# Intsights/PySubstringSearch

Hardware: AMD Instinct MI355X
Metric: queries/sec (batched) + index-build GB/s on 512MB chunk, 1/2/4/8 GPU (higher is better)
Workload: dtype u64

## Files before the change

include/pss.h:

```cpp
#ifndef PSS_H
#define PSS_H

#include <stddef.h>
#include <stdint.h>

#ifdef __cplusplus
extern "C" {
#endif

#define PSS_OK 0
#define PSS_EINVAL (-1)
#define PSS_ENOMEM (-2)
#define PSS_EIO (-3)
#define PSS_ETOOBIG (-4)
#define PSS_EDEVICE (-5)
#define PSS_EFORMAT (-6)

typedef struct pss_writer pss_writer;
typedef struct pss_reader pss_reader;
typedef struct pss_result pss_result;


int pss_device_count(void);

// ... 39 lines not shown
    uint64_t fs_launches[9];
    uint64_t fs_elems[9];
    uint64_t msd;
    uint64_t msd_buckets;
    uint64_t msd_max_bucket;
    uint64_t msd_tiles;
    double msd_ms_g1;
    double msd_ms_g2;
    double msd_ms_local;
    uint64_t msd_slow_tiles;
    uint64_t runs;
    uint64_t rle;
    uint64_t rle_id_bits;
    double rle_ms_table;
    double rle_ms_reduced;
    double rle_ms_expand;
    uint64_t ss;
    uint64_t ss_buckets;
    uint64_t ss_max_bucket;
    uint64_t ss_tiles;
    uint64_t ss_samples;
    double ss_ms_sample;
    double ss_ms_g1;
    double ss_ms_g2;
    double ss_ms_local;
    double ms_initial;
    uint64_t period;
    uint64_t period_extent;
    uint64_t period_path;
    uint64_t plan_hint;
    uint64_t anchor;
    uint64_t anchor_omega;
    uint64_t anchor_w;
    uint64_t anchor_count;
    uint64_t anchor_active;
    uint64_t anchor_depth;
    uint64_t anchor_text_rounds;
    uint64_t anchor_rounds;
    uint64_t anchor_sum_active;
    uint64_t anchor_left;
    uint64_t anchor_levels;
    uint64_t probe_pairs;
    uint64_t probe_same;
    uint64_t periodic_rounds;
    uint64_t periodic_members;
    uint64_t ss_planned;
    uint64_t dup_screen;
    uint64_t ss_plan_refused;
    uint64_t ss_declined_nomem;
    uint64_t anchor_side;
    double anchor_ms;
    double ms_restarts;
    uint64_t msd_lookback;
} pss_sa_stats;

int32_t pss_sa_build(const uint8_t *T, int32_t *SA, int32_t n, int32_t device);

int32_t pss_sa_build_device(const void *d_T, void *d_SA, int32_t n, int32_t device,
                            uint32_t flags, pss_sa_stats *stats);

int32_t pss_sort_pairs_device(void *d_keys, void *d_vals, uint32_t n, int32_t key_bits, int32_t device,
                              double *ms_scatter);


int pss_writer_open(const char *path, int64_t max_chunk_len, int32_t device, pss_writer **out);
#define PSS_FORMAT_STRIPED 0x100
int pss_writer_open_format(const char *path, int64_t max_chunk_len, int32_t device, int32_t format_version,
                           pss_writer **out);
int pss_writer_open_multi(const char *path, int64_t max_chunk_len, const int32_t *devices, int32_t n_devices,
                          int32_t format_version, pss_writer **out);
int pss_writer_add_entry(pss_writer *w, const uint8_t *text, uint64_t len);
int pss_writer_add_file_lines(pss_writer *w, const char *path);
int pss_writer_dump(pss_writer *w);
int pss_writer_finalize(pss_writer *w);
int pss_writer_close(pss_writer *w);
uint64_t pss_writer_chunk_limit(const pss_writer *w);
typedef struct pss_writer_io {
    uint64_t records_mapped;
    uint64_t records_pwritten;
    uint64_t ingest_direct_bytes;
    uint64_t ingest_copied_bytes;
} pss_writer_io;
int pss_writer_io_stats(pss_writer *w, pss_writer_io *out);


int pss_reader_open(const char *path, int32_t device, int32_t shard_index, int32_t shard_count,
                    pss_reader **out);
int pss_reader_open_multi(const char *path, const int32_t *devices, int32_t n_devices, pss_reader **out);
uint64_t pss_reader_part_chunks(const pss_reader *r, uint64_t *counts, uint64_t cap);

int pss_reader_set_auto_residency(pss_reader *r, int32_t on);
int pss_reader_chunk_tiers(const pss_reader *r, uint8_t *tiers, uint64_t cap, uint64_t *auto_moves);
int pss_reader_evict_chunk(pss_reader *r, uint64_t index);
int pss_reader_promote_chunk(pss_reader *r, uint64_t index);
int pss_reader_set_low_latency(pss_reader *r, int32_t on);
int pss_reader_low_latency_stats(const pss_reader *r, uint64_t *launches, uint64_t *served);
#define PSS_ORDER_TEXT 0
#define PSS_ORDER_SA 1
int pss_reader_set_result_order(pss_reader *r, int32_t order);
int32_t pss_reader_result_order(const pss_reader *r);
int pss_reader_create(int32_t device, pss_reader **out);
int pss_reader_add_chunk_device(pss_reader *r, const void *d_text, const void *d_sa, uint32_t n);
int pss_reader_set_chunk_device(pss_reader *r, uint64_t index, const void *d_text, const void *d_sa, uint32_t n);
uint64_t pss_reader_num_chunks(const pss_reader *r);
int pss_reader_residency(const pss_reader *r, uint64_t *hbm_bytes, uint64_t *host_bytes, uint64_t *host_chunks);

// ... 127 lines not shown
```

pysubstringsearch_amd/_ffi.py:

```python
import ctypes
import os

_HERE = os.path.dirname(os.path.abspath(__file__))
LIB_PATH = os.environ.get('PSS_LIBPSS') or os.path.join(_HERE, 'libpss.so')

PSS_OK, PSS_EINVAL, PSS_ENOMEM, PSS_EIO, PSS_ETOOBIG, PSS_EDEVICE, PSS_EFORMAT = 0, -1, -2, -3, -4, -5, -6

CORPUS_LINES, CORPUS_WORDS, CORPUS_RUNS, CORPUS_PERIODIC = 0, 1, 2, 3
CORPUS_REPEAT_LINE, CORPUS_DUP_BLOCKS, CORPUS_MIXED, CORPUS_SOURCE = 4, 5, 6, 7


class SaStats(ctypes.Structure):
    _fields_ = [
        ('sigma', ctypes.c_uint32),
        ('code_bits', ctypes.c_uint32),
        ('key_chars', ctypes.c_uint32),
        ('initial_passes', ctypes.c_uint32),
        ('rounds', ctypes.c_uint32),
        ('round_passes', ctypes.c_uint32),
        ('sum_active', ctypes.c_uint64),
        ('sort_elems', ctypes.c_uint64),
        ('ms_total', ctypes.c_double),
        ('ms_sort', ctypes.c_double),
        ('sort_launches', ctypes.c_uint64),
# ... 10 lines not shown
        ('fs_launches', ctypes.c_uint64 * 9),
        ('fs_elems', ctypes.c_uint64 * 9),
        ('msd', ctypes.c_uint64),
        ('msd_buckets', ctypes.c_uint64),
        ('msd_max_bucket', ctypes.c_uint64),
        ('msd_tiles', ctypes.c_uint64),
        ('msd_ms_g1', ctypes.c_double),
        ('msd_ms_g2', ctypes.c_double),
        ('msd_ms_local', ctypes.c_double),
        ('msd_slow_tiles', ctypes.c_uint64),
        ('runs', ctypes.c_uint64),
        ('rle', ctypes.c_uint64),
        ('rle_id_bits', ctypes.c_uint64),
        ('rle_ms_table', ctypes.c_double),
        ('rle_ms_reduced', ctypes.c_double),
        ('rle_ms_expand', ctypes.c_double),
        ('ss', ctypes.c_uint64),
        ('ss_buckets', ctypes.c_uint64),
        ('ss_max_bucket', ctypes.c_uint64),
        ('ss_tiles', ctypes.c_uint64),
        ('ss_samples', ctypes.c_uint64),
        ('ss_ms_sample', ctypes.c_double),
        ('ss_ms_g1', ctypes.c_double),
        ('ss_ms_g2', ctypes.c_double),
        ('ss_ms_local', ctypes.c_double),
        ('ms_initial', ctypes.c_double),
        ('period', ctypes.c_uint64),
        ('period_extent', ctypes.c_uint64),
        ('period_path', ctypes.c_uint64),
        ('plan_hint', ctypes.c_uint64),
        ('anchor', ctypes.c_uint64),
        ('anchor_omega', ctypes.c_uint64),
        ('anchor_w', ctypes.c_uint64),
        ('anchor_count', ctypes.c_uint64),
        ('anchor_active', ctypes.c_uint64),
        ('anchor_depth', ctypes.c_uint64),
        ('anchor_text_rounds', ctypes.c_uint64),
        ('anchor_rounds', ctypes.c_uint64),
        ('anchor_sum_active', ctypes.c_uint64),
        ('anchor_left', ctypes.c_uint64),
        ('anchor_levels', ctypes.c_uint64),
        ('probe_pairs', ctypes.c_uint64),
        ('probe_same', ctypes.c_uint64),
        ('periodic_rounds', ctypes.c_uint64),
        ('periodic_members', ctypes.c_uint64),
        ('ss_planned', ctypes.c_uint64),
        ('dup_screen', ctypes.c_uint64),
        ('ss_plan_refused', ctypes.c_uint64),
        ('ss_declined_nomem', ctypes.c_uint64),
        ('anchor_side', ctypes.c_uint64),
        ('anchor_ms', ctypes.c_double),
        ('ms_restarts', ctypes.c_double),
        ('msd_lookback', ctypes.c_uint64),
    ]

    def as_dict(self):
        d = {k: getattr(self, k) for k, _ in self._fields_}
        for k in ('fs_ms', 'fs_launches', 'fs_elems'):
            d[k] = list(d[k])
        return d


def knobs():
    out = []
    for i in range(lib.pss_knob_count()):
        f = [ctypes.c_char_p() for _ in range(4)]
        check(lib.pss_knob_info(i, *[ctypes.byref(x) for x in f]))
        name, dflt, fuzz, what = [x.value.decode() for x in f]
        out.append({'name': name, 'default': dflt, 'fuzz': [v for v in fuzz.split('|') if v], 'what': what})
    return out


class SearchStats(ctypes.Structure):
    _fields_ = [
        ('queries', ctypes.c_uint64),
        ('hits', ctypes.c_uint64),
        ('entries', ctypes.c_uint64),
        ('result_bytes', ctypes.c_uint64),
        ('ms_device', ctypes.c_double),
        ('ms_interval', ctypes.c_double),
        ('ms_host', ctypes.c_double),
        ('route', ctypes.c_uint32),
        ('route_pad', ctypes.c_uint32),
    ]

    def as_dict(self):
        return {k: getattr(self, k) for k, _ in self._fields_ if k != 'route_pad'}


ROUTES = {
    'RESIDENT': 0x0001,
    'SMALL_BLOCK': 0x0002,
    'SMALL_WAVE': 0x0004,
    'SMALL_OVERFLOW': 0x0008,
    'INTERVAL_LANE': 0x0010,
    'INTERVAL_GROUP': 0x0020,
    'INTERVAL_WAVE': 0x0040,
    'KEY_SAMPLES': 0x0080,
    'MID': 0x0100,
    'MID_OVERFLOW': 0x0200,
    'GENERAL': 0x0400,
    'SA_ORDER': 0x0800,
    'COUNTS': 0x1000,
    'ANCHORED': 0x2000,
}

# ... 198 lines not shown
```

pysubstringsearch_amd/csrc/common.cpp:

```cpp
#include "common.h"
#include "knobs.h"

#include <atomic>
#include <cstring>
#include <cstdio>
#include <cstdlib>
#include <algorithm>
#include <cerrno>
#include <unistd.h>

#include <mutex>
#include <vector>

namespace pss {

static thread_local std::string g_err;

void set_error(const char *fmt, ...)
{
    char buf[1024];
    va_list ap;
    va_start(ap, fmt);
    vsnprintf(buf, sizeof buf, fmt, ap);
    va_end(ap);
// ... 325 lines not shown
    return PSS_OK;
}

int get_ctx(int device, DeviceCtx **out) { return get_ctx_of(g_ctx, device, out); }
int get_build_ctx(int device, DeviceCtx **out) { return get_ctx_of(g_bctx, device, out); }

int DeviceCtx::ensure_resident()
{
    if (resident.arena) return PSS_OK;
    PSS_HIP(hipStreamCreateWithFlags(&resident.stream, hipStreamNonBlocking));
    PSS_HIP(hipHostMalloc(&resident.arena, kPinnedBytes, hipHostMallocCoherent | hipHostMallocMapped));
    PSS_HIP(hipHostGetDevicePointer(&resident.arena_dev, resident.arena, 0));
    memset(resident.arena, 0, kPinnedBytes);
    return PSS_OK;
}

void DeviceCtx::Resident::post(const uint8_t *q, uint32_t plen)
{
    ResidentMailbox *mb = reinterpret_cast<ResidentMailbox *>(static_cast<uint8_t *>(arena) + kResidentMailboxOff);
    if (plen != kResidentStop) {
        if (plen <= sizeof mb->post.bytes) {
            memcpy(mb->post.bytes, q, plen);
        } else {
            memcpy(mb->query, q, plen);
            memset(mb->query + plen, 0, 32);
        }
    }
    mb->post.plen = plen;
    ++seq;
    __atomic_store_n(&mb->post.seq_b, seq, __ATOMIC_RELEASE);
    __atomic_store_n(&mb->post.seq_a, seq, __ATOMIC_RELEASE);
}

void DeviceCtx::stop_resident()
{
    if (!resident.running) return;
    resident.post(nullptr, kResidentStop);
    (void)hipStreamSynchronize(resident.stream);
    resident.running = false;
}

const KnobDef kKnobs[] = {
    {"PSS_KEY_CHARS", "0 (chosen)", "1|2|3|5|8|12|16", "builder: force the symbols packed into the initial sort key"},
    {"PSS_KEY_DROP", "-1 (chosen)", "0|1|3|7", "builder: force the low bits of the last key symbol that are left out"},
    {"PSS_NO_SAMPLE", "unset", "1", "builder: size the initial key from symbol counts even for large texts (no sizing sample)"},
    {"PSS_NO_TIES_PASS", "unset", "1", "builder: plain 8-byte-key LSD passes and key comparison in the rerank (no tie flags)"},
    {"PSS_MODE", "chosen", "dense|sparse|text", "builder: how ties are resolved -- doubling over an inverse suffix array, sparse (hash), text rounds"},
    {"PSS_TEXT_ROUNDS", "5", "0|1|2|3", "builder: text rounds at most before the rank rounds"},
    {"PSS_MSD", "-1 (screened)", "0|1|1", "initial sort: never / whenever the key fits the hybrid MSD radix sort (msd_sort.hip)"},
    {"PSS_MSD_LSD", "1", "0|1", "MSD sort: 0 = digits in MSD order with a second histogram pass (rounds 2-5); else LSD order, second pass by look-back"},
    {"PSS_MSD_KEY_CAP", "48", "", "MSD sort: largest key width tried (bits; the element format bounds it further)"},
    {"PSS_MSD_PARTIAL_SYMBOL", "unset", "1", "MSD sort: fill the element with the high bits of one more symbol than fits whole (fewer ties; measured slower on lines)"},
    {"PSS_MSD_NO_FUSE", "unset", "1", "MSD sort: ties flagged in the suffix array instead of emitted from the local sort"},
    {"PSS_MSD_SLOW_LOCAL", "unset", "1", "MSD sort: the general (ballot LSD) local-sort kernel for every tile"},
    {"PSS_MSD_SCATTER", "unset", "1", "MSD sort in MSD order: the 8192-element partition kernels of round 2"},
    {"PSS_SS", "-1 (n >= 2^24, MSD declined)", "0|1", "initial sort: never / whenever the text has the size for it the sample sort over 16-byte elements"},
    {"PSS_SS_SEG", "1", "0", "sample sort: 0 = every tile merge-sorted as one array instead of bucket by bucket"},
    {"PSS_SS_WINDOW_PLAN", "unset", "1", "sample sort: tiles by the window rule of the MSD sort instead of the greedy plan"},
    {"PSS_SS_DEBUG", "unset", "", "sample sort: print where a bucket beyond a tile came from (diagnostic)"},
    {"PSS_NO_PLAN_CACHE", "unset", "1", "builder: forget between chunks which initial sort and alphabet the previous chunk took"},
    {"PSS_NO_PLAN_FRONT", "unset", "1", "builder: remember the sort but not the alphabet (separate alphabet and recode passes)"},
    {"PSS_RLE", "-1 (runs average >= 8 bytes)", "0|1|1", "builder: never / always the run-length path (rle_build.hip)"},
    {"PSS_RLE_SORT", "unset", "1", "run-length path: expansion by the stable radix sort instead of the matrix walk"},
    {"PSS_PERIOD", "-1 (when the text repeats one word)", "0", "builder: 0 = never the closed form for a text that repeats one word"},
    {"PSS_ANCHOR", "-1 (texts of >= 2^20 bytes)", "0|1|1", "builder: never / whenever ties outlive the text rounds the anchor round (anchor_impl.h)"},
    {"PSS_ANCHOR_OMEGA", "0 (as wide as the common prefix allows)", "9|12|17|33", "anchor round: force the window of the minimizers"},
    {"PSS_ANCHOR_MIN_OMEGA", "11", "3|7|9", "anchor round: narrowest window it accepts by itself"},
    {"PSS_ANCHOR_SIDE", "-1 (>= 2^24 bytes, sampled ties show copies)", "0|1", "anchor round: never / always sort the anchors beside the text round (second stream)"},
    {"PSS_ANCHOR_SIDE_PCT", "8", "", "anchor round: share of sampled tied pairs that must be copies for the side line"},
    {"PSS_ANCHOR_CAP_DIV", "5", "3|4", "anchor round: declines above n / this many anchors"},
    {"PSS_NO_PROBE", "unset", "1", "builder: always a text round before the anchor round (no sampling of the ties)"},
    {"PSS_PROBE_SKIP_PCT", "50", "0|20|90", "builder: no text rounds when more than this share of the sampled tied pairs are repeats"},
    {"PSS_NO_MID_TIER", "unset", "1", "rounds: groups above 512 members all take the chained radix sorts"},
    {"PSS_NO_MID_MERGE", "unset", "1", "rounds: groups of 513 .. 4096 members with a crowded bin take the chained sorts (no LDS merge sort)"},
    {"PSS_BIG_MERGE", "-1 (by the average size of the large groups)", "0|1|2", "rounds: groups above 4096 members through the segmented merge sort (2: in text rounds only)"},
    {"PSS_NO_BIG_MERGE", "unset", "", "rounds: overrides PSS_BIG_MERGE"},
    {"PSS_COUNT_SORT", "unset", "1", "rank rounds: groups ranked by counting instead of the merge sort"},
    {"PSS_PERIODIC", "1", "0", "rank rounds: 0 = no periodic keys for the large groups"},
    {"PSS_TIMING", "unset", "", "builder / Writer: per-round and per-stage trace on stderr"},
    {"PSS_DEVICES", "all visible", "0|0,0|0,0,0|all", "devices of Reader(path) / Writer(path) without a device argument: all | comma-separated ordinals"},
    {"PSS_DEVICE", "unset", "", "default device of a process (launchers' LOCAL_RANK etc. are honoured the same way)"},
    {"PSS_IO_THREADS", "8 .. 16 by core count", "2|5", "file path: threads of the I/O pool"},
    {"PSS_INGEST_BLOCK", "32 MiB", "16|40|300", "Writer: size of the direct reads of add_entries_from_file_lines"},
    {"PSS_INGEST_MIN_ROOM", "1 MiB", "1|20", "Writer: room a chunk must have left for one direct read"},
    {"PSS_WRITER_MMAP", "tmpfs: 1, else 0", "0|1", "Writer: records through a shared mapping (1) or pwrite (0)"},
    {"PSS_WRITER_MMAP_MIN", "1 MiB", "16", "Writer: smallest record that goes through the mapping"},
    {"PSS_WRITER_HOST_BUDGET", "8 GiB", "", "multi-device Writer: host text of the chunks in flight (one chunk always goes through)"},
    {"PSS_STRIPES", "8", "", "striped container format 2: stripe files of a Writer"},
    {"PSS_EXPERIMENT_NO_FILE", "unset", "", "measurement only: the record thread copies without writing the file"},
    {"PSS_RESULT_ORDER", "text", "sa", "Reader: 'sa' = the reference's order inside a chunk (suffix-array order of every entry's first hit)"},
    {"PSS_READER_HBM_BUDGET", "whatever hipMalloc grants minus 2 GiB", "", "Reader: suffix arrays beyond this many bytes of HBM stay in pinned host memory"},
    {"PSS_READER_AUTO_RESIDENCY", "1", "", "Reader: 0 = the residency manager never moves a suffix array by itself"},
    {"PSS_NO_KEY_SAMPLES", "unset", "", "Reader: no key-sample table"},
    {"PSS_SAMPLE_SHIFT", "11", "", "Reader: one key sample per 2^shift suffixes"},
    {"PSS_LINE_BLOCK_SHIFT", "8", "6|7|9|10", "Reader: the line index behind entry ids keeps one newline rank per 2^shift bytes of text (6 .. 10)"},
    {"PSS_NO_SMALL_PATH", "unset", "1", "search: no fused single-query kernels"},
    {"PSS_NO_BLOCK_PATH", "unset", "1", "search: small batches one wave per pair instead of one workgroup"},
    {"PSS_NO_SEARCH_STAGE", "unset", "1", "search: no pinned staging of queries and results"},
    {"PSS_WAVE_SEARCH", "unset", "1", "search: interval kernel one wave per pair at every batch size"},
    {"PSS_NO_GROUP_SEARCH", "unset", "1", "search: never 16 lanes per pair"},
    {"PSS_NO_MID_PIPELINE", "unset", "1", "search: always the general multi-kernel pipeline"},
    {"PSS_PINNED_POOL_BYTES", "40 GiB", "", "search: pinned host memory the result pool keeps between batches"},
    {"PSS_NO_PINNED_RESULTS", "unset", "1", "search: large results into pageable memory"},
    {"PSS_LANE_SEARCH_MIN", "8192", "1|100000", "search: pairs from which one lane per pair searches"},
    {"PSS_ICASE_SEED_LETTERS", "5", "1|2|3|4|5|6", "case-insensitive search: ASCII letters of a pattern's seed at most (2^letters spellings probed per pattern and chunk)"},
    {"PSS_SEARCH_EVENTS", "unset", "", "single-query path: HIP events around the fused kernel (fills ms_device; ~4 us per query)"},
// ... 58 lines not shown
```

pysubstringsearch_amd/csrc/msd_sort.h:

```cpp
#pragma once
#include "common.h"
#include "radix_sort.h"

namespace pss {

struct MsdStats {
    uint32_t buckets = 0;
    uint32_t max_bucket = 0;
    uint32_t tiles = 0;
    uint32_t slow_tiles = 0;
    uint32_t bad_symbol = 0;
    uint32_t lookback = 0;
    double ms_g1 = 0, ms_g2 = 0, ms_local = 0;
};

struct MsdActive {
    uint32_t *pos, *idx, *grp;
    uint32_t *st_pos, *st_idx;
    uint32_t count = 0;
};

size_t msd_workspace_bytes(uint32_t n);
int msd_max_key_bits(uint32_t n);

struct MsdFront {
    const uint8_t *raw;
    const uint8_t *lut;
    uint32_t *bad;
};
int msd_suffix_sort(DeviceCtx *ctx, const TextKeys *text, uint32_t n, int key_bits, uint64_t *A[2], uint32_t *sa_out,
                    void *work, uint32_t *h_small, bool profile, MsdStats *stats, bool *accepted, MsdActive *active = nullptr,
                    const MsdFront *front = nullptr);


struct SsStats {
    uint32_t buckets = 0, max_bucket = 0, tiles = 0;
    uint32_t b1 = 0, b2 = 0, samples = 0;
    int key_chars = 0;
    double ms_sample = 0, ms_g1 = 0, ms_g2 = 0, ms_local = 0;
};
struct SsBuffers {
    void *A[2];
    uint16_t *digits;
    void *E0, *E;
    uint64_t *K[2];
    uint32_t *V[2];
    void *sort_work;
    const void *sample_in = nullptr;
    void *sample_keep = nullptr;
};
uint32_t ss_sample_count(uint32_t n);
int ss_key_chars(uint32_t n, uint32_t radix);
uint64_t ss_geometry_tag(uint32_t n, uint32_t radix);
int ss_suffix_sort(DeviceCtx *ctx, const TextKeys *text, uint32_t radix, uint32_t n, const SsBuffers &buf, uint32_t *sa_out,
                   void *work, uint32_t *h_small, bool profile, SsStats *stats, bool *accepted, MsdActive *active);

}
```

pysubstringsearch_amd/csrc/msd_sort.hip:

```cpp
#include "msd_sort.h"

#include <algorithm>
#include <vector>

#include "prims.h"
#include "scan.h"
#include "text_keys.h"

namespace pss {

constexpr int MSD_D = 10;
constexpr u32 MSD_BINS = 1u << MSD_D;
constexpr int MSD_BLOCK = 512;
constexpr int MSD_WAVES = MSD_BLOCK / kWave;
constexpr int MSD_IPT = 16;
constexpr u32 MSD_TILE = MSD_BLOCK * MSD_IPT;
constexpr u32 MSD_WIN = 6144;
#ifndef PSS_LS_WINDOW
#define PSS_LS_WINDOW 8
#endif
constexpr u32 MSD_TILE_CAP = 8184 - PSS_LS_WINDOW;
constexpr u32 MSD_MAX_BUCKET = 4088;
constexpr int MSD_TAG_BITS = MSD_D + 1;
constexpr u32 MSD_TAG_SPAN = 1u << MSD_TAG_BITS;
// ... 752 lines not shown
}

__global__ __launch_bounds__(256) void msd_tiles_kernel(const u32 *cstart, u32 ne, u32 n, const u64 *rank, const u64 *total,
                                                          u32 *tile_first, TilePlan tp)
{
    if (blockIdx.x == 0 && threadIdx.x == 0) tile_first[*total] = ne;
    for (u32 k = blockIdx.x * blockDim.x + threadIdx.x; k < ne; k += gridDim.x * blockDim.x) {
        if (msd_tile_head(cstart, ne, n, k, tp)) tile_first[rank[k]] = k;
    }
}

struct MsdTile {
    u32 e0, count, tag0, nb;
};


struct MsdEmit {
    u32 *st_pos, *st_idx;
    u32 *blk_cnt;
};

__device__ __forceinline__ void msd_emit_tile(const u64 *exch, u32 count, u32 e0, int idx_bits, u32 *sa_out, const MsdEmit *em,
                                              u32 *s_count)
{
    const u32 tid = threadIdx.x, lane = tid & 63u;
    const u32 imask = (u32)((1ull << idx_bits) - 1ull);
    const u32 rows = (count + MSD_BLOCK - 1) / MSD_BLOCK;
#pragma unroll 1
    for (u32 r = 0; r < rows; ++r) {
        const u32 p = r * MSD_BLOCK + tid;
        const bool valid = p < count;
        u64 x = 0;
        bool tie = false;
        if (valid) {
            x = exch[p];
            tie = p > 0 && (exch[p - 1] >> idx_bits) == (x >> idx_bits);
            sa_out[e0 + p] = ((u32)x & imask) | ((tie && em == nullptr) ? 0x80000000u : 0u);
        }
        if (em != nullptr) {
            const u64 tm = __ballot(tie);
            const bool tie_next = lane < 63 ? ((tm >> (lane + 1)) & 1ull) != 0
                                            : (p + 1 < count && (exch[p + 1] >> idx_bits) == (x >> idx_bits));
            if (valid && (tie || tie_next)) {
                const u32 slot = e0 + atomicAdd(s_count, 1u);
                em->st_pos[slot] = e0 + p;
                em->st_idx[slot] = ((u32)x & imask) | (tie ? 0x80000000u : 0u);
            }
        }
    }
}

struct InBlkCnt {
    const u32 *c;
    __device__ u64 operator()(u64 t) const { return c[t]; }
};

constexpr u32 GA_WORDS = MSD_TILE / 32;
__global__ __launch_bounds__(256) void msd_gather_kernel(const MsdTile *tiles, const u32 *blk_cnt, const u64 *dst_off, u32 nt,
                                                           const u32 *st_pos, const u32 *st_idx, u32 *pos, u32 *idx, u32 *grp)
{
    __shared__ u32 s_occ[4][GA_WORDS], s_head[4][GA_WORDS], s_pre[4][GA_WORDS];
    const u32 w = wave_id(), lane = lane_id();
    const u32 t = blockIdx.x * 4 + w;
    if (t >= nt) return;
    const u32 c = blk_cnt[t];
    if (c == 0) return;
    const u32 e0 = tiles[t].e0;
    const u64 d = dst_off[t];
    u32 *occ = s_occ[w], *head = s_head[w], *pre = s_pre[w];
    for (u32 i = lane; i < GA_WORDS; i += kWave) occ[i] = head[i] = 0;
    __builtin_amdgcn_fence(__ATOMIC_ACQ_REL, "wavefront");
    __builtin_amdgcn_wave_barrier();
    for (u32 i = lane; i < c; i += kWave) {
        const u32 q = st_pos[e0 + i] - e0;
        atomicOr(&occ[q >> 5], 1u << (q & 31u));
        if (!(st_idx[e0 + i] >> 31)) atomicOr(&head[q >> 5], 1u << (q & 31u));
    }
    __builtin_amdgcn_fence(__ATOMIC_ACQ_REL, "wavefront");
    __builtin_amdgcn_wave_barrier();
    {
        const u32 c0 = __popc(occ[4 * lane]), c1 = __popc(occ[4 * lane + 1]), c2 = __popc(occ[4 * lane + 2]),
                  c3 = __popc(occ[4 * lane + 3]);
        const u32 ex = wave_incl_sum(c0 + c1 + c2 + c3) - (c0 + c1 + c2 + c3);
        pre[4 * lane] = ex;
        pre[4 * lane + 1] = ex + c0;
        pre[4 * lane + 2] = ex + c0 + c1;
        pre[4 * lane + 3] = ex + c0 + c1 + c2;
    }
    __builtin_amdgcn_fence(__ATOMIC_ACQ_REL, "wavefront");
    __builtin_amdgcn_wave_barrier();
    for (u32 i = lane; i < c; i += kWave) {
        const u32 ps = st_pos[e0 + i], q = ps - e0;
        const u32 below = (q & 31u) ? (occ[q >> 5] & ((1u << (q & 31u)) - 1u)) : 0u;
        const u32 rank = pre[q >> 5] + __popc(below);
        u32 wi = q >> 5;
        u32 m = head[wi] & ((q & 31u) == 31u ? ~0u : ((2u << (q & 31u)) - 1u));
        while (m == 0 && wi > 0) m = head[--wi];
        const u32 hq = wi * 32 + (31u - (u32)__builtin_clz(m | 1u));
        pos[d + rank] = ps;
        idx[d + rank] = st_idx[e0 + i] & 0x7fffffffu;
        grp[d + rank] = e0 + hq + 1;
    }
}


__global__ __launch_bounds__(MSD_BLOCK) void msd_local_sort_kernel(const u64 *in, const MsdTile *tiles, int rem_bits, int idx_bits,
                                                                     u32 *sa_out, const u32 *tile_list, int fused, MsdEmit em_val)
{
    const MsdEmit *em = fused ? &em_val : nullptr;
    __shared__ __attribute__((aligned(16))) u64 exch[MSD_TILE];
    __shared__ u32 wave_hist[MSD_WAVES][256];
    __shared__ u32 scr[MSD_WAVES + 1];
    const u32 tid = threadIdx.x, lane = tid & 63u, wave = tid >> 6;
    const u32 t = tile_list ? tile_list[blockIdx.x] : blockIdx.x;
    const MsdTile td = tiles[t];
    const u32 e0 = td.e0, count = td.count;
    for (u32 i = tid; i < MSD_WAVES * 256; i += MSD_BLOCK) (&wave_hist[0][0])[i] = 0;
    __syncthreads();
    int seg_bits = 0;
    while ((1u << seg_bits) < td.nb) ++seg_bits;
    const u64 tag_base = (u64)td.tag0 << (rem_bits + idx_bits);
    u64 key[MSD_IPT];
#pragma unroll
    for (int r = 0; r < MSD_IPT; ++r) {
        const u32 p = wave * (kWave * MSD_IPT) + r * kWave + lane;
        key[r] = p < count ? in[e0 + p] - tag_base : ~0ull;
    }
    const int sort_bits = rem_bits + seg_bits;
    for (int shift = idx_bits; shift < idx_bits + sort_bits; shift += 8) {
        const int left = idx_bits + sort_bits - shift;
        const u32 dmask = left >= 8 ? 0xffu : ((1u << left) - 1u);
        u32 rank[MSD_IPT], prev[MSD_IPT];
#pragma unroll
        for (int r = 0; r < MSD_IPT; ++r) {
            const bool pad = wave * (kWave * MSD_IPT) + r * kWave + lane >= count;
            const u32 d = pad ? dmask : ((u32)(key[r] >> shift) & dmask);
            const u64 peers = match_digit8(d, ~0ull);
            const u32 below = mbcnt(peers);
            prev[r] = 0;
            if (below == 0) prev[r] = atomicAdd(&wave_hist[wave][d], (u32)__popcll(peers));
            rank[r] = below | ((u32)__builtin_ctzll(peers) << 16);
        }
#pragma unroll
        for (int r = 0; r < MSD_IPT; ++r) rank[r] = __shfl(prev[r], (int)(rank[r] >> 16)) + (rank[r] & 0xffffu);
        __syncthreads();
        {
            u32 c[MSD_WAVES];
            u32 total = 0;
            if (tid < 256) {
#pragma unroll
                for (int w = 0; w < MSD_WAVES; ++w) {
                    c[w] = wave_hist[w][tid];
                    total += c[w];
                }
            }
// ... 514 lines not shown
        else hipLaunchKernelGGL(msd_scatter_kernel<false>, dim3((u32)max_ranges2), dim3(MSD_BLOCK), 0, s, a);
        PSS_TRY(mark());
    }
    const auto local_sort = msd_local_sort_kernel;
    const auto local_fast = msd_local_fast_kernel;
    u32 nt = 0;
    u32 *fail_list = fail_list_dev;
    if (one_trip) {
        nt = h_small[8];
        if ((size_t)nt > max_tiles) {
            set_error("msd_suffix_sort: %u tiles planned, tables hold %zu (internal error)", nt, max_tiles);
            return PSS_EDEVICE;
        }
        const u32 nfail = h_small[10];
        if (stats) stats->slow_tiles = nfail;
        if (nfail)
            hipLaunchKernelGGL(local_sort, dim3(nfail), dim3(MSD_BLOCK), 0, s, A[1], (const MsdTile *)tiles_all, rem_bits,
                               ib, sa_out, (const u32 *)fail_list, fused, em);
    } else {
    const TilePlan tp{MSD_WIN, MSD_TILE_CAP, cj};
    PSS_TRY(device_excl_scan(ctx, InTileHead{cstart, ne, n, tp}, ne, partial, d_total, ranks));
    hipLaunchKernelGGL(msd_tiles_kernel, dim3(1024), dim3(256), 0, s, cstart, ne, n, ranks, (const u64 *)d_total, tile_first, tp);
    PSS_HIP(hipMemcpyAsync(h_small, d_total, 8, hipMemcpyDeviceToHost, s));
    PSS_HIP(hipStreamSynchronize(s));
    nt = h_small[0];
    if ((size_t)nt > max_tiles) {
        set_error("msd_suffix_sort: %u tiles planned, tables hold %zu (internal error)", nt, max_tiles);
        return PSS_EDEVICE;
    }
    PSS_TRY(mark());
    fail_list = tile_first + nt + 8;
    hipLaunchKernelGGL(msd_tile_desc_kernel, dim3((nt + 255) / 256), dim3(256), 0, s, cstart, tile_first, nt, ne, n, tiles_all,
                       (const u32 *)cj, (const u64 *)nullptr, (const u64 *)nullptr);
    if (knob("PSS_MSD_SLOW_LOCAL")) {
        hipLaunchKernelGGL(local_sort, dim3(nt), dim3(MSD_BLOCK), 0, s, A[1], (const MsdTile *)tiles_all, rem_bits, ib,
                           sa_out, (const u32 *)nullptr, fused, em);
    } else {
        MsdTile *tiles = tiles_all;
        const u32 grid = std::min<u32>(nt, 2u * (u32)ctx->num_cus);
        hipLaunchKernelGGL(local_fast, dim3(grid), dim3(MSD_BLOCK), 0, s, A[1], (const MsdTile *)tiles, nt, rem_bits, ib,
                           sa_out, fail_list, counters + 4, fused, em, (const u64 *)nullptr, (const u32 *)nullptr, (const u32 *)nullptr);
        PSS_TRY(mark());
        PSS_HIP(hipMemcpyAsync(h_small, counters + 4, 4, hipMemcpyDeviceToHost, s));
        PSS_HIP(hipStreamSynchronize(s));
        const u32 nfail = h_small[0];
        if (stats) stats->slow_tiles = nfail;
        if (nfail)
            hipLaunchKernelGGL(local_sort, dim3(nfail), dim3(MSD_BLOCK), 0, s, A[1], (const MsdTile *)tiles_all, rem_bits,
                               ib, sa_out, (const u32 *)fail_list, fused, em);
    }
    if (knob("PSS_MSD_SLOW_LOCAL")) PSS_TRY(mark());
    }
    if (fused) {
        PSS_TRY(device_excl_scan(ctx, InBlkCnt{blk_cnt}, nt, partial, d_total, dst_off));
        hipLaunchKernelGGL(msd_gather_kernel, dim3((nt + 3) / 4), dim3(256), 0, s, (const MsdTile *)tiles_all, blk_cnt, dst_off, nt,
                           active->st_pos, active->st_idx, active->pos, active->idx, active->grp);
        PSS_HIP(hipMemcpyAsync(h_small, d_total, 8, hipMemcpyDeviceToHost, s));
        PSS_HIP(hipStreamSynchronize(s));
        active->count = h_small[0];
    }
    PSS_HIP(hipGetLastError());
    if (stats) {
        stats->tiles = nt;
        stats->lookback = lsd ? 1u : 0u;
    }
    if (profile && nev >= 6) {
        PSS_HIP(hipStreamSynchronize(s));
        float ms = 0.f;
        PSS_HIP(hipEventElapsedTime(&ms, ev[0], ev[1]));
        if (stats) stats->ms_g1 = ms;
        PSS_HIP(hipEventElapsedTime(&ms, ev[2], ev[3]));
        if (stats) stats->ms_g2 = ms;
        PSS_HIP(hipEventElapsedTime(&ms, ev[4], ev[5]));
        if (stats) stats->ms_local = ms;
    }
    *accepted = true;
    return PSS_OK;
}


struct SsGeometry {
    u32 B1, B2, os, S;
    int ib, kc, key_bits;
    u64 plo, phi;
};
static bool ss_geometry(uint32_t n, uint32_t radix, SsGeometry *g)
{
    if (n < (1u << 16) || n > (1u << 30) || radix < 2 || radix > 257) return false;
    int ib = 1;
    while ((1ull << ib) < (u64)n) ++ib;
    const unsigned __int128 limit = (unsigned __int128)1 << (128 - ib);
    unsigned __int128 pw = 1;
    int kc = 0;
    while (kc < SS_MAX_CHARS && pw <= limit / radix) {
        pw *= radix;
        ++kc;
    }
    if (kc < 2) return false;
    unsigned __int128 lead = 1;
    for (int i = 0; i + 1 < kc; ++i) lead *= radix;
    g->plo = (u64)lead;
    g->phi = (u64)(lead >> 64);
    int kb = 0;
    while (kb < 128 && ((pw - 1) >> kb) != 0) ++kb;
    g->key_bits = kb;
    int lb = 4;
    while (((u64)512 << lb) < (u64)n && lb < 20) ++lb;
    const u32 B1 = 1u << ((lb + 1) / 2), B2 = 1u << (lb / 2);
    const u32 os = ((u64)n > (u64)768 * B1 * B2) ? 8u : 4u;
    g->B1 = B1;
    g->B2 = B2;
    g->os = os;
// ... 245 lines not shown
```

pysubstringsearch_amd/csrc/sa_build.hip:

```cpp
#include "prims.h"
#include "msd_sort.h"
#include "rle_build.h"
#include "radix_sort.h"
#include "sa_build.h"
#include "scan.h"
#include "anchor_impl.h"

#include <algorithm>
#include <cmath>
#include <string>
#include <thread>

namespace pss {


constexpr u32 DUP_SAMPLES = 8192, DUP_SLOTS = 16384;
__global__ __launch_bounds__(1024) void dup_screen_kernel(const u8 *T, u32 n, u32 *dups)
{
    __shared__ u32 table[DUP_SLOTS];
    for (u32 i = threadIdx.x; i < DUP_SLOTS; i += 1024) table[i] = 0;
    __syncthreads();
    u32 mine = 0;
    if (n >= 64) {
        const u32 stride = (n - 32) / DUP_SAMPLES;
        for (u32 k = threadIdx.x; k < DUP_SAMPLES; k += 1024) {
            u64 x = ((u64)k + 1) * 0x9E3779B97F4A7C15ull;
            x ^= x >> 29;
            x *= 0xBF58476D1CE4E5B9ull;
            x ^= x >> 32;
            const u32 pos = stride ? k * stride + (u32)(x % stride) : k % (n - 32);
            const u64 a = load_u64_unaligned(T + pos), b = load_u64_unaligned(T + pos + 8);
            u64 hsh = (a ^ (b * 0x9E3779B97F4A7C15ull)) * 0xD6E8FEB86659FD93ull;
            hsh ^= hsh >> 32;
            u32 f = (u32)hsh;
            if (f == 0) f = 1;
            u32 slot = (f * 2654435761u) >> (32 - 14);
            static_assert(DUP_SLOTS == (1u << 14), "14-bit slot");
            for (;;) {
                const u32 old = atomicCAS(&table[slot], 0u, f);
                if (old == 0u) break;
                if (old == f) { ++mine; break; }
                slot = (slot + 1) & (DUP_SLOTS - 1);
            }
        }
    }
    const u32 tot = wave_incl_sum(mine);
    if (lane_id() == kWave - 1 && tot) atomicAdd(dups, tot);
}

__global__ __launch_bounds__(256) void sa_symbols_kernel(const u8 *T, u32 n, u32 *present, u32 *counts, u32 *runs)
{
    __shared__ u32 seen[256];
    __shared__ u32 cnt[256];
    const u32 tid = threadIdx.x;
    seen[tid] = 0;
    cnt[tid] = 0;
    u32 nruns = 0;
    __syncthreads();
// ... 368 lines not shown
    const int passes0 = (key_bits0 + 7) / 8;
    const int final_buf = (passes0 - 1) & 1;
    u32 *const v_scratch = V[final_buf];
    V[final_buf] = SA;
    int cur = 0;
    const bool ties = passes0 >= 2 && !knobs.no_flags;
    bool msd_done = false, msd_fused = false;
    u32 msd_active = 0;
    if (ties && knobs.msd != 0) {
        const char *cap_env = knob("PSS_MSD_KEY_CAP");
        const int key_cap = cap_env ? atoi(cap_env) : 48;
        const bool whole = knob("PSS_MSD_PARTIAL_SYMBOL") == nullptr;
        int kb = std::min(msd_max_key_bits(n), std::max(key_cap, 21));
        int kc = std::min(whole ? kb / b : (kb + b - 1) / b, kmax);
        int mdrop = kc * b - kb;
        if (mdrop < 0 || kc <= 1) {
            kb = kc * b;
            mdrop = 0;
        }
        const bool fits = kc >= 1 && kb >= 21 && !plus_one;
        const bool auto_ok = sampled && msd_screen_ok && (hint == 1 || (key_bits0 <= 48 && kb + 8 >= key_bits0));
        if (fits && (knobs.msd == 1 || (knobs.msd < 0 && auto_ok))) {
            TextKeys mk{codes, b, kc, plus_one, mdrop};
            MsdStats ms;
            bool accepted = false;
            PSS_TRY(ctx->slot[S_GRP2].reserve((size_t)n * 4));
            MsdActive act;
            act.pos = ctx->slot[S_P1].as<u32>();
            act.idx = (final_buf == 0) ? V[1] : V[0];
            act.grp = ctx->slot[S_GRP2].as<u32>();
            act.st_pos = reinterpret_cast<u32 *>(K[0]);
            act.st_idx = reinterpret_cast<u32 *>(K[0]) + n;
            const MsdFront front{T, d_lut, d_bad};
            PSS_TRY(msd_suffix_sort(ctx, &mk, n, kb, K, SA, ctx->slot[S_P0].p, h_small, profile, &ms, &accepted,
                                    knobs.no_msd_fuse ? nullptr : &act, front_any ? &front : nullptr));
            if (front_any && !accepted) {
                ctx->plan_path = 0;
                return start_over(fresh ? (flags | 4u) : flags);
            }
            msd_fused = accepted && !knobs.no_msd_fuse;
            msd_active = act.count;
            st.msd_buckets = ms.buckets;
            st.msd_max_bucket = ms.max_bucket;
            if (accepted) {
                msd_done = true;
                key_chars = kc;
                key_drop = mdrop;
                st.key_chars = (u32)kc;
                st.key_bits = (u64)kb;
                st.msd = 1;
                st.msd_tiles = ms.tiles;
                st.msd_slow_tiles = ms.slow_tiles;
                st.msd_lookback = ms.lookback;
                st.msd_ms_g1 = ms.ms_g1;
                st.msd_ms_g2 = ms.ms_g2;
                st.msd_ms_local = ms.ms_local;
                cur = final_buf;
                ss.launches = 3;
                ss.elems = 3ull * n;
            }
        }
    }
    if (front_any && !msd_done) {
        ctx->plan_path = 0;
        return start_over(fresh ? (flags | 4u) : flags);
    }
    if (!msd_done && ties && knobs.ss != 0 && (knobs.ss == 1 || (n >= (1u << 24) && !forced_chars && knobs.key_chars == 0)) &&
        ss_sample_count(n) != 0) {
        const u32 S = ss_sample_count(n);
        bool ss_room = ctx->slot[S_SSA].reserve((size_t)n * 16 + 256) == PSS_OK && ctx->slot[S_SSB].reserve((size_t)n * 16 + 256) == PSS_OK;
        if (!ss_room) {
            (void)hipGetLastError();
            ctx->slot[S_SSA].release();
            ctx->slot[S_SSB].release();
            set_error("%s", "");
            st.ss_declined_nomem = 1;
        }
        if (ss_room) {
        PSS_TRY(ctx->slot[S_GRP2].reserve((size_t)n * 4));
        SsBuffers sb;
        sb.A[0] = ctx->slot[S_SSA].p;
        sb.A[1] = ctx->slot[S_SSB].p;
        sb.digits = reinterpret_cast<uint16_t *>(ctx->slot[S_P1].p);
        sb.E0 = GRP;
        sb.E = ISA;
        sb.K[0] = K[0]; sb.K[1] = K[1];
        sb.V[0] = v_scratch; sb.V[1] = (final_buf == 0) ? V[1] : V[0];
        sb.sort_work = work;
        const u32 radix = plus_one ? 257u : sigma + 1u;
        const u64 tag = ss_geometry_tag(n, radix);
        const bool planned = hint == 2 && tag != 0 && ctx->ss_plan_tag == tag && ctx->ss_plan_radix == radix && ctx->slot[S_SSPLAN].p != nullptr &&
                             ctx->ss_plan_skip == 0;
        if (planned) sb.sample_in = ctx->slot[S_SSPLAN].p;
        else if (plain && ctx->slot[S_SSPLAN].reserve((size_t)S * 16) == PSS_OK) sb.sample_keep = ctx->slot[S_SSPLAN].p;
        ctx->ss_plan_tag = 0;
        MsdActive act;
        act.pos = ctx->slot[S_P1].as<u32>();
        act.idx = (final_buf == 0) ? V[1] : V[0];
        act.grp = ctx->slot[S_GRP2].as<u32>();
        act.st_pos = reinterpret_cast<u32 *>(K[0]);
        act.st_idx = reinterpret_cast<u32 *>(K[0]) + n;
        TextKeys sk{codes, b, 0, plus_one, 0};
        SsStats sst;
        bool accepted = false;
        PSS_TRY(ss_suffix_sort(ctx, &sk, plus_one ? 257u : sigma + 1u, n, sb, SA, ctx->slot[S_P0].p, h_small, profile, &sst, &accepted,
                               &act));
// ... 111 lines not shown
```

pysubstringsearch_amd/csrc/sa_rerank_impl.h:

```cpp


constexpr int RR_BLOCK = 256;
constexpr int RR_WAVES = RR_BLOCK / kWave;
#ifndef PSS_RR_ROWS
#define PSS_RR_ROWS 8
#endif
constexpr int RR_ROWS = PSS_RR_ROWS;
constexpr int RR_WSEG = RR_ROWS * kWave;
constexpr int RR_TILE = RR_WSEG * RR_WAVES;
constexpr u32 RR_MAX_RANGES = 1024;

struct RerankArgs {
    const u64 *keys;
    const u32 *idx;
    const u32 *pos;
    const u32 *grp;
    const u32 *tied_sa;
    u32 m;
    u32 num_tiles, tiles_per_range, num_ranges;
    u32 *agg_head;
    u32 *agg_cnt;
    u32 *SA;
    u32 *ISA;
    u32 *pos_out, *idx_out, *grp_out;
// ... 357 lines not shown
        if (lane == 0) { s_wh[w] = whead; s_wc[w] = wcnt; }
        __syncthreads();
        u32 carry_h = s_carry_h, carry_c = s_carry_c;
        u32 tile_h = carry_h, tile_c = carry_c;
#pragma unroll
        for (int k = 0; k < RR_WAVES; ++k) {
            if (k < (int)w) { carry_h = max(carry_h, s_wh[k]); carry_c += s_wc[k]; }
            tile_h = max(tile_h, s_wh[k]);
            tile_c += s_wc[k];
        }
        __syncthreads();
        if (threadIdx.x == 0) { s_carry_h = tile_h; s_carry_c = tile_c; }
        if (wcnt == 0) continue;
#pragma unroll
        for (int hf = 0; hf < 2; ++hf) {
            if (lane_cnt[hf] == 0) continue;
            const u64 j = wbase + 256u * hf + 4u * lane;
            u32 u = carry_c + excl_c[hf];
            u32 hd1 = max(carry_h, excl_h[hf]);
#pragma unroll
            for (int c = 0; c < 4; ++c) {
                if (j + c < m) {
                    const u32 x = v[hf][c];
                    if (!(x >> 31)) hd1 = (u32)(j + c) + 1u;
                    const u32 tn = (c < 3) ? v[hf][c + 1] : nxt[hf];
                    const bool next_tied = (j + c + 1 < m) && (tn >> 31);
                    if ((x >> 31) || next_tied) {
                        a.pos_out[u] = (u32)(j + c);
                        a.idx_out[u] = x & 0x7fffffffu;
                        a.grp_out[u] = hd1;
                        ++u;
                    }
                }
            }
        }
    }
}

struct KeyArgs {
    const u32 *idx;
    const u32 *grp;
    const u32 *ISA;
    const u64 *ht;
    u32 ht_mask;
    const u32 *sa;
    const u8 *codes;
    int code_bits, key_chars, plus_one;
    u32 m, n, h;
    int rank_bits;
    u64 *keys;
    u64 *red;
};

__device__ __forceinline__ u64 text_key_at(const u8 *codes, u32 j, int b, int k, int plus_one, u32 n)
{
    const uint4 *q = reinterpret_cast<const uint4 *>(codes + (j & ~15u));
    const uint4 a = q[0], c = q[1];
    const u64 x0 = (u64)a.x | ((u64)a.y << 32), x1 = (u64)a.z | ((u64)a.w << 32);
    const u64 x2 = (u64)c.x | ((u64)c.y << 32), x3 = (u64)c.z | ((u64)c.w << 32);
    const bool up = (j & 8u) != 0;
    const u32 s8 = (j & 7u) * 8u;
    const u64 l0 = up ? x1 : x0, l1 = up ? x2 : x1, l2 = up ? x3 : x2;
    const u64 w0 = s8 ? (l0 >> s8) | (l1 << (64 - s8)) : l0;
    const u64 w1 = s8 ? (l1 >> s8) | (l2 << (64 - s8)) : l1;
    u64 key = 0;
#pragma unroll
    for (int c = 0; c < 16; ++c) {
        if (c < k) {
            u32 v = (u32)((c < 8 ? w0 : w1) >> ((c & 7) * 8)) & 0xffu;
            if (plus_one) v = ((u64)j + c < n) ? v + 1u : 0u;
            key = (key << b) | v;
        }
    }
    return key;
}

template <bool SPARSE>
__global__ __launch_bounds__(256) void build_keys_kernel(KeyArgs a)
{
    u64 vor = 0, vand = ~0ull;
    for (u32 t = blockIdx.x * blockDim.x + threadIdx.x; t < a.m; t += gridDim.x * blockDim.x) {
        const u64 i2 = (u64)a.idx[t] + a.h;
        u32 r2 = 0;
        if (i2 < a.n) {
            if (SPARSE) {
                r2 = ht_lookup(a.ht, a.ht_mask, (u32)i2);
                if (r2 == 0) {
                    const u64 key = text_key_at(a.codes, (u32)i2, a.code_bits, a.key_chars, a.plus_one, a.n);
                    u32 lo = 0, hi = a.n;
                    while (lo < hi) {
                        const u32 mid = lo + ((hi - lo) >> 1);
                        if (text_key_at(a.codes, a.sa[mid] & 0x7fffffffu, a.code_bits, a.key_chars, a.plus_one, a.n) < key) lo = mid + 1;
                        else hi = mid;
                    }
                    r2 = lo + 1;
                }
            } else {
                r2 = a.ISA[i2];
            }
        }
        const u64 key = ((u64)a.grp[t] << a.rank_bits) | r2;
        a.keys[t] = key;
        vor |= key;
        vand &= key;
    }
#pragma unroll
    for (int o = 32; o > 0; o >>= 1) {
        vor |= __shfl_xor(vor, o);
        vand &= __shfl_xor(vand, o);
    }
    __shared__ u64 s_or[256 / kWave], s_and[256 / kWave];
    if (lane_id() == 0) {
        s_or[wave_id()] = vor;
        s_and[wave_id()] = vand;
    }
    __syncthreads();
    if (threadIdx.x == 0) {
#pragma unroll
        for (int w = 1; w < 256 / kWave; ++w) {
            vor |= s_or[w];
            vand &= s_and[w];
        }
        atomicOr(reinterpret_cast<unsigned long long *>(&a.red[0]), (unsigned long long)vor);
        atomicAnd(reinterpret_cast<unsigned long long *>(&a.red[1]), (unsigned long long)vand);
    }
}
```

pysubstringsearch_amd/csrc/text_keys.h:

```cpp
#pragma once
#include "prims.h"

namespace pss {

constexpr int TK_IPT = 16;

__device__ __forceinline__ void text_keys16(const u8 *codes, u32 i0, int b, int k, int plus_one, int drop, u32 n,
                                            u64 (&key)[TK_IPT])
{
    const uint4 *p = reinterpret_cast<const uint4 *>(codes + i0);
    const uint4 lo = p[0], hi = p[1];
    const u64 q0 = (u64)lo.x | ((u64)lo.y << 32), q1 = (u64)lo.z | ((u64)lo.w << 32);
    const u64 q2 = (u64)hi.x | ((u64)hi.y << 32), q3 = (u64)hi.z | ((u64)hi.w << 32);
    const u64 mask = (k * b >= 64) ? ~0ull : ((1ull << (k * b)) - 1ull);
    u64 win = 0;
#pragma unroll
    for (int j = 0; j < 16; ++j) {
        const u64 src = (j < 8) ? q0 : q1;
        u32 c = (u32)(src >> ((j & 7) * 8)) & 0xffu;
        if (plus_one) c = (i0 + j < n) ? c + 1u : 0u;
        if (j < k) win = (win << b) | c;
    }
    key[0] = win >> drop;
    u64 a0, a1, a2;
    if (k >= 16) { a0 = q2; a1 = q3; a2 = 0; }
    else if (k >= 8) { a0 = q1; a1 = q2; a2 = q3; }
    else { a0 = q0; a1 = q1; a2 = q2; }
    const int sh = (k & 7) * 8;
    u64 s0 = a0, s1 = a1;
    if (sh) {
        s0 = (a0 >> sh) | (a1 << (64 - sh));
        s1 = (a1 >> sh) | (a2 << (64 - sh));
    }
#pragma unroll
    for (int r = 1; r < TK_IPT; ++r) {
        const int j = r - 1;
        const u64 src = (j < 8) ? s0 : s1;
        u32 c = (u32)(src >> ((j & 7) * 8)) & 0xffu;
        if (plus_one) c = ((u64)i0 + j + k < n) ? c + 1u : 0u;
        win = ((win << b) | c) & mask;
        key[r] = win >> drop;
    }
}

}
```

Baseline: 66.21.

## Finish small MSD tie groups with one extra text key after local sort

Adds a kernel that runs after the fused MSD local sort. It finds tie groups of up to four suffixes, compares one more text key at the following offset, and writes their final order straight into the suffix array when the keys differ. Those groups are then dropped from the active set, so fewer elements go into the later doubling or text rounds. The sparse rank lookup is adjusted to skip over settled neighbours. The costs are an extra kernel launch, packed counters in blk_cnt, and a risk of rank inconsistency in sparse mode.

Result: faster. 67.31, median of 6 (+1.7%).

```diff
diff --git a/include/pss.h b/include/pss.h
--- a/include/pss.h
+++ b/include/pss.h
@@ -115,6 +115,7 @@
     double anchor_ms;
     double ms_restarts;
     uint64_t msd_lookback;
+    uint64_t msd_finished;
 } pss_sa_stats;
 
 int32_t pss_sa_build(const uint8_t *T, int32_t *SA, int32_t n, int32_t device);
diff --git a/pysubstringsearch_amd/_ffi.py b/pysubstringsearch_amd/_ffi.py
--- a/pysubstringsearch_amd/_ffi.py
+++ b/pysubstringsearch_amd/_ffi.py
@@ -86,6 +86,7 @@
         ('anchor_ms', ctypes.c_double),
         ('ms_restarts', ctypes.c_double),
         ('msd_lookback', ctypes.c_uint64),
+        ('msd_finished', ctypes.c_uint64),
     ]
 
     def as_dict(self):
diff --git a/pysubstringsearch_amd/csrc/common.cpp b/pysubstringsearch_amd/csrc/common.cpp
--- a/pysubstringsearch_amd/csrc/common.cpp
+++ b/pysubstringsearch_amd/csrc/common.cpp
@@ -401,6 +401,7 @@
     {"PSS_MSD_KEY_CAP", "48", "", "MSD sort: largest key width tried (bits; the element format bounds it further)"},
     {"PSS_MSD_PARTIAL_SYMBOL", "unset", "1", "MSD sort: fill the element with the high bits of one more symbol than fits whole (fewer ties; measured slower on lines)"},
     {"PSS_MSD_NO_FUSE", "unset", "1", "MSD sort: ties flagged in the suffix array instead of emitted from the local sort"},
+    {"PSS_MSD_NO_FINISH", "unset", "1", "MSD sort: small tie groups go to the rounds instead of being finished by one more text key after the local sort"},
     {"PSS_MSD_SLOW_LOCAL", "unset", "1", "MSD sort: the general (ballot LSD) local-sort kernel for every tile"},
     {"PSS_MSD_SCATTER", "unset", "1", "MSD sort in MSD order: the 8192-element partition kernels of round 2"},
     {"PSS_SS", "-1 (n >= 2^24, MSD declined)", "0|1", "initial sort: never / whenever the text has the size for it the sample sort over 16-byte elements"},
diff --git a/pysubstringsearch_amd/csrc/msd_sort.h b/pysubstringsearch_amd/csrc/msd_sort.h
--- a/pysubstringsearch_amd/csrc/msd_sort.h
+++ b/pysubstringsearch_amd/csrc/msd_sort.h
@@ -11,9 +11,11 @@
     uint32_t slow_tiles = 0;
     uint32_t bad_symbol = 0;
     uint32_t lookback = 0;
+    uint32_t finished = 0;
     double ms_g1 = 0, ms_g2 = 0, ms_local = 0;
 };
 
+constexpr int MSD_FIN_MAX = 4;
 struct MsdActive {
     uint32_t *pos, *idx, *grp;
     uint32_t *st_pos, *st_idx;
diff --git a/pysubstringsearch_amd/csrc/msd_sort.hip b/pysubstringsearch_amd/csrc/msd_sort.hip
--- a/pysubstringsearch_amd/csrc/msd_sort.hip
+++ b/pysubstringsearch_amd/csrc/msd_sort.hip
@@ -828,7 +828,7 @@
 
 struct InBlkCnt {
     const u32 *c;
-    __device__ u64 operator()(u64 t) const { return c[t]; }
+    __device__ u64 operator()(u64 t) const { return (u64)(c[t] & 0xffffu) | ((u64)(c[t] >> 16) << 32); }
 };
 
 constexpr u32 GA_WORDS = MSD_TILE / 32;
@@ -839,10 +839,10 @@
     const u32 w = wave_id(), lane = lane_id();
     const u32 t = blockIdx.x * 4 + w;
     if (t >= nt) return;
-    const u32 c = blk_cnt[t];
+    const u32 c = blk_cnt[t] & 0xffffu;
     if (c == 0) return;
     const u32 e0 = tiles[t].e0;
-    const u64 d = dst_off[t];
+    const u64 d = dst_off[t] & 0xffffffffull;
     u32 *occ = s_occ[w], *head = s_head[w], *pre = s_pre[w];
     for (u32 i = lane; i < GA_WORDS; i += kWave) occ[i] = head[i] = 0;
     __builtin_amdgcn_fence(__ATOMIC_ACQ_REL, "wavefront");
@@ -877,6 +877,122 @@
         idx[d + rank] = st_idx[e0 + i] & 0x7fffffffu;
         grp[d + rank] = e0 + hq + 1;
     }
+}
+
+
+constexpr int FIN_MAX = MSD_FIN_MAX;
+constexpr u32 FIN_WORDS = GA_WORDS + 2;
+struct MsdFinish {
+    const u8 *codes;
+    int code_bits, key_syms, plus_one;
+    u32 h0, n;
+};
+
+__global__ __launch_bounds__(256) void msd_finish_kernel(const MsdTile *tiles, u32 *blk_cnt, u32 nt, u32 *st_pos, u32 *st_idx,
+                                                           u32 *sa_out, MsdFinish f)
+{
+    __shared__ u32 s_tie[4][FIN_WORDS], s_done[4][GA_WORDS];
+    const u32 w = wave_id(), lane = lane_id();
+    const u32 t = blockIdx.x * 4 + w;
+    if (t >= nt) return;
+    const u32 c = blk_cnt[t] & 0xffffu;
+    const u32 e0 = tiles[t].e0;
+    if (c == 0) return;
+    u32 ps0 = 0, v0 = 0;
+    if (lane < c) {
+        ps0 = st_pos[e0 + lane];
+        v0 = st_idx[e0 + lane];
+    }
+    auto record = [&](u32 i, u32 &ps, u32 &v) {
+        if (i < (u32)kWave) {
+            ps = ps0;
+            v = v0;
+        } else {
+            ps = st_pos[e0 + i];
+            v = st_idx[e0 + i];
+        }
+    };
+    u32 *tie = s_tie[w], *done = s_done[w];
+    for (u32 i = lane; i < FIN_WORDS; i += kWave) tie[i] = 0;
+    for (u32 i = lane; i < GA_WORDS; i += kWave) done[i] = 0;
+    __builtin_amdgcn_fence(__ATOMIC_ACQ_REL, "wavefront");
+    __builtin_amdgcn_wave_barrier();
+    for (u32 i = lane; i < c; i += kWave) {
+        u32 ps, v;
+        record(i, ps, v);
+        const u32 q = ps - e0;
+        if (v >> 31) atomicOr(&tie[q >> 5], 1u << (q & 31u));
+    }
+    __builtin_amdgcn_fence(__ATOMIC_ACQ_REL, "wavefront");
+    __builtin_amdgcn_wave_barrier();
+    bool settled = false;
+    for (u32 i = lane; i < c; i += kWave) {
+        u32 ps, v;
+        record(i, ps, v);
+        if (v >> 31) continue;
+        const u32 q = ps - e0, a = q + 1u;
+        const u64 win = (((u64)tie[(a >> 5) + 1u] << 32) | (u64)tie[a >> 5]) >> (a & 31u);
+        const u32 g = win == ~0ull ? 65u : 1u + (u32)__builtin_ctzll(~win);
+        if (g > (u32)FIN_MAX) continue;
+        u32 sfx[FIN_MAX], rk[FIN_MAX];
+        u64 key[FIN_MAX];
+#pragma unroll
+        for (int j = 0; j < FIN_MAX; ++j) {
+            sfx[j] = 0;
+            key[j] = 0;
+            rk[j] = 0;
+            if ((u32)j < g) {
+                sfx[j] = j == 0 ? v : sa_out[ps + j];
+                const u64 at = (u64)sfx[j] + f.h0;
+                if (at < f.n) key[j] = text_key_at(f.codes, (u32)at, f.code_bits, f.key_syms, f.plus_one, f.n);
+            }
+        }
+        bool same = false;
+#pragma unroll
+        for (int j = 0; j < FIN_MAX; ++j) {
+#pragma unroll
+            for (int l = j + 1; l < FIN_MAX; ++l) {
+                if ((u32)l < g) {
+                    same |= key[j] == key[l];
+                    rk[l] += key[j] < key[l] ? 1u : 0u;
+                    rk[j] += key[j] < key[l] ? 0u : 1u;
+                }
+            }
+        }
+        if (same) continue;
+        settled = true;
+#pragma unroll
+        for (int j = 0; j < FIN_MAX; ++j) {
+            if ((u32)j < g) {
+                sa_out[ps + rk[j]] = sfx[j];
+                atomicOr(&done[(q + j) >> 5], 1u << ((q + j) & 31u));
+            }
+        }
+    }
+    __builtin_amdgcn_fence(__ATOMIC_ACQ_REL, "wavefront");
+    __builtin_amdgcn_wave_barrier();
+    if (__ballot(settled) == 0) return;
+    u32 kept = 0;
+    for (u32 base = 0; base < c; base += kWave) {
+        const u32 i = base + lane;
+        u32 ps = 0, v = 0;
+        bool keep = false;
+        if (i < c) {
+            record(i, ps, v);
+            const u32 q = ps - e0;
+            keep = ((done[q >> 5] >> (q & 31u)) & 1u) == 0;
+        }
+        const u64 km = __ballot(keep);
+        __builtin_amdgcn_fence(__ATOMIC_ACQ_REL, "wavefront");
+        __builtin_amdgcn_wave_barrier();
+        if (keep) {
+            const u32 o = e0 + kept + mbcnt(km);
+            st_pos[o] = ps;
+            st_idx[o] = v;
+        }
+        kept += (u32)__popcll(km);
+    }
+    if (lane == 0) blk_cnt[t] = kept | ((c - kept) << 16);
 }
 
 
@@ -1497,12 +1613,21 @@
     if (knob("PSS_MSD_SLOW_LOCAL")) PSS_TRY(mark());
     }
     if (fused) {
+        const bool finish = knob("PSS_MSD_NO_FINISH") == nullptr;
+        if (finish) {
+            const int ks = std::min(64 / text->code_bits, 16);
+            const MsdFinish fin{text->codes, text->code_bits, ks, text->plus_one,
+                                (u32)(text->drop ? text->key_chars - 1 : text->key_chars), n};
+            hipLaunchKernelGGL(msd_finish_kernel, dim3((nt + 3) / 4), dim3(256), 0, s, (const MsdTile *)tiles_all, blk_cnt, nt,
+                               active->st_pos, active->st_idx, sa_out, fin);
+        }
         PSS_TRY(device_excl_scan(ctx, InBlkCnt{blk_cnt}, nt, partial, d_total, dst_off));
         hipLaunchKernelGGL(msd_gather_kernel, dim3((nt + 3) / 4), dim3(256), 0, s, (const MsdTile *)tiles_all, blk_cnt, dst_off, nt,
                            active->st_pos, active->st_idx, active->pos, active->idx, active->grp);
         PSS_HIP(hipMemcpyAsync(h_small, d_total, 8, hipMemcpyDeviceToHost, s));
         PSS_HIP(hipStreamSynchronize(s));
         active->count = h_small[0];
+        if (stats) stats->finished = h_small[1];
     }
     PSS_HIP(hipGetLastError());
     if (stats) {
diff --git a/pysubstringsearch_amd/csrc/sa_build.hip b/pysubstringsearch_amd/csrc/sa_build.hip
--- a/pysubstringsearch_amd/csrc/sa_build.hip
+++ b/pysubstringsearch_amd/csrc/sa_build.hip
@@ -4,6 +4,7 @@
 #include "radix_sort.h"
 #include "sa_build.h"
 #include "scan.h"
+#include "text_keys.h"
 #include "anchor_impl.h"
 
 #include <algorithm>
@@ -478,6 +479,7 @@
                 st.msd_tiles = ms.tiles;
                 st.msd_slow_tiles = ms.slow_tiles;
                 st.msd_lookback = ms.lookback;
+                st.msd_finished = ms.finished;
                 st.msd_ms_g1 = ms.ms_g1;
                 st.msd_ms_g2 = ms.ms_g2;
                 st.msd_ms_local = ms.ms_local;
diff --git a/pysubstringsearch_amd/csrc/sa_rerank_impl.h b/pysubstringsearch_amd/csrc/sa_rerank_impl.h
--- a/pysubstringsearch_amd/csrc/sa_rerank_impl.h
+++ b/pysubstringsearch_amd/csrc/sa_rerank_impl.h
@@ -433,28 +433,6 @@
     u64 *red;
 };
 
-__device__ __forceinline__ u64 text_key_at(const u8 *codes, u32 j, int b, int k, int plus_one, u32 n)
-{
-    const uint4 *q = reinterpret_cast<const uint4 *>(codes + (j & ~15u));
-    const uint4 a = q[0], c = q[1];
-    const u64 x0 = (u64)a.x | ((u64)a.y << 32), x1 = (u64)a.z | ((u64)a.w << 32);
-    const u64 x2 = (u64)c.x | ((u64)c.y << 32), x3 = (u64)c.z | ((u64)c.w << 32);
-    const bool up = (j & 8u) != 0;
-    const u32 s8 = (j & 7u) * 8u;
-    const u64 l0 = up ? x1 : x0, l1 = up ? x2 : x1, l2 = up ? x3 : x2;
-    const u64 w0 = s8 ? (l0 >> s8) | (l1 << (64 - s8)) : l0;
-    const u64 w1 = s8 ? (l1 >> s8) | (l2 << (64 - s8)) : l1;
-    u64 key = 0;
-#pragma unroll
-    for (int c = 0; c < 16; ++c) {
-        if (c < k) {
-            u32 v = (u32)((c < 8 ? w0 : w1) >> ((c & 7) * 8)) & 0xffu;
-            if (plus_one) v = ((u64)j + c < n) ? v + 1u : 0u;
-            key = (key << b) | v;
-        }
-    }
-    return key;
-}
 
 template <bool SPARSE>
 __global__ __launch_bounds__(256) void build_keys_kernel(KeyArgs a)
@@ -474,6 +452,7 @@
                         if (text_key_at(a.codes, a.sa[mid] & 0x7fffffffu, a.code_bits, a.key_chars, a.plus_one, a.n) < key) lo = mid + 1;
                         else hi = mid;
                     }
+                    for (int s = 1; s < MSD_FIN_MAX && lo + 1 < a.n && (a.sa[lo] & 0x7fffffffu) != (u32)i2; ++s) ++lo;
                     r2 = lo + 1;
                 }
             } else {
diff --git a/pysubstringsearch_amd/csrc/text_keys.h b/pysubstringsearch_amd/csrc/text_keys.h
--- a/pysubstringsearch_amd/csrc/text_keys.h
+++ b/pysubstringsearch_amd/csrc/text_keys.h
@@ -43,4 +43,27 @@
     }
 }
 
+__device__ __forceinline__ u64 text_key_at(const u8 *codes, u32 j, int b, int k, int plus_one, u32 n)
+{
+    const uint4 *q = reinterpret_cast<const uint4 *>(codes + (j & ~15u));
+    const uint4 a = q[0], c = q[1];
+    const u64 x0 = (u64)a.x | ((u64)a.y << 32), x1 = (u64)a.z | ((u64)a.w << 32);
+    const u64 x2 = (u64)c.x | ((u64)c.y << 32), x3 = (u64)c.z | ((u64)c.w << 32);
+    const bool up = (j & 8u) != 0;
+    const u32 s8 = (j & 7u) * 8u;
+    const u64 l0 = up ? x1 : x0, l1 = up ? x2 : x1, l2 = up ? x3 : x2;
+    const u64 w0 = s8 ? (l0 >> s8) | (l1 << (64 - s8)) : l0;
+    const u64 w1 = s8 ? (l1 >> s8) | (l2 << (64 - s8)) : l1;
+    u64 key = 0;
+#pragma unroll
+    for (int c = 0; c < 16; ++c) {
+        if (c < k) {
+            u32 v = (u32)((c < 8 ? w0 : w1) >> ((c & 7) * 8)) & 0xffu;
+            if (plus_one) v = ((u64)j + c < n) ? v + 1u : 0u;
+            key = (key << b) | v;
+        }
+    }
+    return key;
 }
+
+}
```
